# meilisearch/arroy

Hardware: AMD Instinct MI355X
Metric: distances/sec, Q=1 batched 768-dim cosine scan (GB/s vs HBM roofline in `roofline`); tree-build seconds at 10M vectors in `build_10m` (higher is better)
Workload: dtype f32; 1 GPU; 1M x 768 cosine Q=1 scan (configs[1])

## Files before the change

arroy_amd/_lib.py:

```python
from __future__ import annotations

import ctypes as C
import os
import subprocess

HERE = os.path.dirname(os.path.abspath(__file__))
LIB_PATH = os.environ.get("AH_LIB_PATH") or os.path.join(HERE, "libarroy_hip.so")
CSRC = os.path.join(HERE, "csrc")

AH_OK = 0
STATUS_NAMES = {
    1: "InvalidVecDimension", 2: "BuildCancelled", 3: "Panic(device)", 4: "Panic(out of memory)",
    5: "Panic(invalid argument)", 6: "MissingKey", 7: "Panic(not finalized)", 8: "Panic(need preprocess)",
}
AH_SPLIT_SAMPLES = 12


class ArroyHipError(RuntimeError):
    def __init__(self, status: int, message: str, detail=None):
        super().__init__(f"{STATUS_NAMES.get(status, status)}: {message}")
        self.status = status
        self.message = message
        self.item = detail.item if detail is not None else 0
        self.expected = detail.expected if detail is not None else 0
# ... 93 lines not shown

NODE_BATCH_FN = C.CFUNCTYPE(C.c_int, C.c_void_p, C.POINTER(AhNodeBatch))


_VP, _U32P, _F32P, _U64P = C.c_void_p, C.c_void_p, C.c_void_p, C.c_void_p
SIGNATURES = {
    "ah_header_size": (C.c_size_t, [C.c_int]),
    "ah_vector_size": (C.c_size_t, [C.c_int, C.c_uint32]),
    "ah_abi_version": (C.c_int, []),
    "ah_device_count": (C.c_int, [C.POINTER(C.c_int)]),
    "ah_last_error": (C.c_char_p, []),
    "ah_last_error_detail": (C.c_int, [C.POINTER(AhErrorDetail)]),
    "ah_dataset_upload_flush": (C.c_int, [_VP]),
    "ah_dataset_set_preprocessed": (C.c_int, [_VP, C.c_int]),
    "ah_dataset_replicate": (C.c_int, [_VP, C.c_int, C.POINTER(C.c_void_p)]),
    "ah_dataset_create": (C.c_int, [C.c_int, C.c_uint32, C.c_uint64, C.c_int, C.POINTER(C.c_void_p)]),
    "ah_dataset_upload_records": (C.c_int, [_VP, _U32P, _VP, C.c_size_t, C.c_size_t]),
    "ah_dataset_upload_vectors": (C.c_int, [_VP, _U32P, _F32P, C.c_size_t]),
    "ah_dataset_fill_synthetic": (C.c_int, [_VP, C.c_uint64, C.c_int, C.c_uint64]),
    "ah_dataset_finalize": (C.c_int, [_VP]),
    "ah_dataset_reserve_build": (C.c_int, [_VP, C.c_uint32, C.c_uint32]),
    "ah_dataset_rerank_stats": (C.c_int, [_VP, C.POINTER(AhRerankStats), C.c_int]),
    "ah_dataset_packed_info": (C.c_int, [_VP, C.POINTER(C.c_int), C.POINTER(C.c_uint64)]),
    "ah_debug_query_screen_verify": (C.c_int, [_VP, C.POINTER(C.c_uint64), C.POINTER(C.c_uint64), C.c_int]),
    "ah_dataset_len": (C.c_int, [_VP, C.POINTER(C.c_uint64)]),
    "ah_dataset_item_vector": (C.c_int, [_VP, C.c_uint32, _F32P]),
    "ah_dataset_read_headers": (C.c_int, [_VP, C.c_uint64, C.c_uint64, _VP]),
    "ah_dataset_destroy": (C.c_int, [_VP]),
    "ah_preprocess_dot": (C.c_int, [_VP, C.POINTER(C.c_float)]),
    "ah_distances_by_vector": (C.c_int, [_VP, _F32P, _U32P, C.c_size_t, _F32P]),
    "ah_distances_by_item": (C.c_int, [_VP, C.c_uint32, _U32P, C.c_size_t, _F32P]),
    "ah_rerank_by_vector": (C.c_int, [_VP, _F32P, _U32P, C.c_size_t, C.c_size_t, _U32P, _F32P,
                                      C.POINTER(C.c_size_t)]),
    "ah_rerank_by_item": (C.c_int, [_VP, C.c_uint32, _U32P, C.c_size_t, C.c_size_t, _U32P, _F32P,
                                    C.POINTER(C.c_size_t)]),
    "ah_rerank_batch": (C.c_int, [_VP, _F32P, C.c_size_t, _U32P, _U64P, C.c_size_t, _U32P, _F32P, _U32P]),
    "ah_split_sides": (C.c_int, [_VP, _VP, _VP, _U32P, C.c_size_t, _VP, C.POINTER(C.c_uint64), _F32P]),
    "ah_margins": (C.c_int, [_VP, _VP, _VP, _U32P, C.c_size_t, _F32P]),
    "ah_create_split": (C.c_int, [_VP, _U32P, _VP, _VP]),
    "ah_build_forest": (C.c_int, [_VP, C.POINTER(AhBuildOptions), C.POINTER(C.c_void_p)]),
    "ah_build_forest_stream": (C.c_int, [_VP, C.POINTER(AhBuildOptions), NODE_BATCH_FN, _VP, _U32P, C.POINTER(AhBuildStats)]),
    "ah_build_subtrees": (C.c_int, [_VP, C.POINTER(AhBuildOptions), _U32P, _U64P, C.POINTER(C.c_void_p)]),
    "ah_forest_view_get": (C.c_int, [_VP, C.POINTER(AhForestView)]),
    "ah_forest_stats": (C.c_int, [_VP, C.POINTER(AhBuildStats)]),
    "ah_forest_digest": (C.c_int, [_VP, _U64P, C.POINTER(C.c_uint64)]),
    "ah_host_cache_trim": (C.c_int, [C.POINTER(C.c_uint64)]),
# ... 171 lines not shown
```

arroy_amd/csrc/api.hip:

```cpp
#include <algorithm>
#include <atomic>
#include <chrono>
#include <cmath>
#include <condition_variable>
#include <functional>
#include <immintrin.h>
#include <new>
#include <thread>
#include <cctype>
#include <cstdio>
#include <mutex>
#include <vector>
#include <sched.h>
#include <sys/syscall.h>
#include <unistd.h>

#include "common.h"

namespace ah {

static thread_local std::string g_error;
static thread_local ah_error_detail g_detail = {AH_OK, 0, 0, 0};

static thread_local int g_guard_depth = 0;
// ... 2249 lines not shown
    AH_GUARDED_END
}

int ah_dataset_rerank_stats(ah_dataset *ds, ah_rerank_stats *out, int reset) {
    AH_GUARDED("ah_dataset_rerank_stats")
    AH_REQUIRE(ds, AH_ERR_INVALID_ARGUMENT, "dataset is NULL");
    std::lock_guard<std::mutex> lk(ds->mu);
    if (out) *out = ds->rr_stats;
    if (reset) ds->rr_stats = ah_rerank_stats{};
    return AH_OK;
    AH_GUARDED_END
}

int ah_dataset_packed_info(ah_dataset *ds, int *out_present, uint64_t *out_raw_rows) {
    AH_GUARDED("ah_dataset_packed_info")
    AH_REQUIRE(ds, AH_ERR_INVALID_ARGUMENT, "dataset is NULL");
    std::lock_guard<std::mutex> lk(ds->mu);
    if (out_present) *out_present = ds->d_packed ? 1 : 0;
    if (out_raw_rows) *out_raw_rows = ds->d_packed ? ds->packed_raw_rows : 0;
    return AH_OK;
    AH_GUARDED_END
}

int ah_debug_query_screen_verify(ah_dataset *ds, uint64_t *out_checked, uint64_t *out_violations, int reset) {
    AH_GUARDED("ah_debug_query_screen_verify")
    AH_REQUIRE(ds, AH_ERR_INVALID_ARGUMENT, "dataset is NULL");
    DeviceRestore restore;
    std::lock_guard<std::mutex> lk(ds->mu);
    unsigned long long c[2] = {0ull, 0ull};
    if (ds->d_query_verify) {
        AH_HIP(hipSetDevice(ds->device));
        AH_HIP(hipDeviceSynchronize());
        AH_HIP(hipMemcpy(c, ds->d_query_verify, 16, hipMemcpyDeviceToHost));
        if (reset) AH_HIP(hipMemset(ds->d_query_verify, 0, 16));
    }
    if (out_checked) *out_checked = c[0];
    if (out_violations) *out_violations = c[1];
    return AH_OK;
    AH_GUARDED_END
}

int ah_split_sides(ah_dataset *ds, const void *normal_vector, const void *normal_header, const uint32_t *sorted_ids,
                   size_t n, uint8_t *side_bits, uint64_t *out_n_left, float *out_margins) {
    AH_GUARDED("ah_split_sides")
    AH_NEED_FINALIZED(ds);
    AH_REQUIRE(normal_vector && normal_header && side_bits && out_n_left, AH_ERR_INVALID_ARGUMENT, "NULL argument");
// ... 233 lines not shown
```

arroy_amd/csrc/common.h:

```cpp
#pragma once

#include <hip/hip_runtime.h>

#include <cstdarg>
#include <cstdint>
#include <cstdio>
#include <atomic>
#include <cstring>
#include <mutex>
#include <new>
#include <string>
#include <thread>
#include <vector>

#include "../../include/arroy_hip.h"
#include "../../include/arroy_hip_policy.h"

namespace ah {

void set_error(const char *fmt, ...);
const char *last_error();
void set_error_status(int status);
void set_error_detail(uint32_t item, uint64_t expected, uint64_t received);

// ... 74 lines not shown
    X(SCREEN_VERIFY, "AH_SCREEN_VERIFY", 0)       \
    X(NODE_PREFETCH, "AH_NODE_PREFETCH", 1)         \
    X(SCREEN8_LO, "AH_SCREEN8_LO", 1)                 \
    X(SCREEN8, "AH_SCREEN8", -1)                 \
    X(MASK_BITS, "AH_MASK_BITS", -1)             \
    X(DENSE, "AH_DENSE", -1)                        \
    X(DENSE_MAX_COLS, "AH_DENSE_MAX_COLS", 16384)                                                                        \
    X(DENSE_NARROW, "AH_DENSE_NARROW", -1)               \
    X(DENSE_NARROW_MAX_COLS, "AH_DENSE_NARROW_MAX_COLS", 64)    \
    X(DENSE_NARROW_STREAM, "AH_DENSE_NARROW_STREAM", 0)  \
    X(DENSE_GMACS, "AH_DENSE_GMACS", 495000)           \
    X(MARGIN_MODE, "AH_MARGIN_MODE", 0)                          \
    X(READBACK_DIRECT, "AH_READBACK_DIRECT", 0)              \
    X(READBACK_PRIORITY, "AH_READBACK_PRIORITY", 1)  \
    X(READBACK_MB, "AH_READBACK_MB", 256)        \
    X(NUMA, "AH_NUMA", 1)                        \
    X(RETRY_GATE, "AH_RETRY_GATE", 1)            \
    X(TAIL_GROUPS, "AH_BUILD_TAIL_GROUPS", 5)    \
    X(TAIL_MIN_MB, "AH_BUILD_TAIL_MIN_MB", 64)   \
    X(TAIL_NODE_ITEMS, "AH_BUILD_TAIL_NODE_ITEMS", 2)  \
    X(TAIL_RATIO, "AH_BUILD_TAIL_RATIO", 76)     \
    X(SCAN_BLOCKS, "AH_SCAN_BLOCKS", 0)                                 \
    X(SCAN_PACKED, "AH_SCAN_PACKED", -1)         \
    X(MANHATTAN_ROWS, "AH_MANHATTAN_ROWS", 1)                                                                            \
    X(RERANK_INVERT, "AH_RERANK_INVERT", -1)          \
    X(RERANK_SMALL, "AH_RERANK_SMALL", 1)        \
    X(PAIR_GROUP, "AH_PAIR_GROUP", 0)                                                                                    \
    X(PAIR_RUNS, "AH_PAIR_RUNS", 1)                                                                                      \
    X(SEARCH_BITMAP, "AH_SEARCH_BITMAP", 1)          \
    X(SEARCH_TILES, "AH_SEARCH_TILES", 1)                          \
    X(SEARCH_WAVE, "AH_SEARCH_WAVE", 1)                        \
    X(SEARCH_BLOCK_MAX_QUERIES, "AH_SEARCH_BLOCK_MAX_QUERIES", 64)  \
    X(SEARCH_SMALL_GATE, "AH_SEARCH_SMALL_GATE", 1)  \
    X(SEARCH_SMALL_UNITS_MAX_QUERIES, "AH_SEARCH_SMALL_UNITS_MAX_QUERIES", 64)  \
    X(SEARCH_FUSED_FLAG, "AH_SEARCH_FUSED_FLAG", 1)  \
    X(SEARCH_FUSED_PREPARE, "AH_SEARCH_FUSED_PREPARE", 1)  \
    X(SEARCH_SINGLE_FUSED, "AH_SEARCH_SINGLE_FUSED", 1)  \
    X(SEARCH_SMALL_TILES_MAX_QUERIES, "AH_SEARCH_SMALL_TILES_MAX_QUERIES", 8)  \
    X(SEARCH_MULTI, "AH_SEARCH_MULTI", 1)        \
    X(SEARCH_MULTI_TREES_PER_BLOCK, "AH_SEARCH_MULTI_TREES_PER_BLOCK", 8)  \
    X(SEARCH_MULTI_IDS_BY_TILES, "AH_SEARCH_MULTI_IDS_BY_TILES", 1)  \
    X(SEARCH_SPIN_WAIT, "AH_SEARCH_SPIN_WAIT", 1)  \
    X(SEARCH_FLAT_TILES, "AH_SEARCH_FLAT_TILES", 1)  \
    X(SEARCH_STATUS_WIPE, "AH_SEARCH_STATUS_WIPE", 1)  \
    X(SEARCH_ITEM_LIST, "AH_SEARCH_ITEM_LIST", 1)  \
    X(SEARCH_MULTI_OWN_UNITS, "AH_SEARCH_MULTI_OWN_UNITS", 1)  \
// ... 76 lines not shown
    float *headers;
    const uint32_t *ids;
    const uint32_t *lut;
    uint32_t lut_len;
    int identity_ids;
};

struct ScreenView {
    const uint16_t *rows;
    const float4 *stats;
    uint32_t hpitch;
    float gamma_s, gamma_r;
    float4 max_stats;
    const int8_t *rows8;
    uint32_t pitch8;
    const float *scale8_rows;
    float4 max8;
    const int8_t *rows8_lo;
    float4 max8b;
};

static constexpr uint16_t kPackedRaw = 0xFFu;
static constexpr uint16_t kPackedZeros = 0x100u;
struct PackedView {
    const uint8_t *rows = nullptr;
    const uint16_t *row_exp = nullptr;
    uint32_t pitch = 0;
    uint32_t hi_off = 0, code_off = 0;
};
inline PackedView packed_layout(uint32_t dims) {
    const uint32_t b = dims / 32;
    PackedView pk;
    pk.hi_off = 128u * ((b + 1) / 2);
    pk.code_off = pk.hi_off + 128u * ((b + 3) / 4);
    pk.pitch = pk.code_off + 128u * ((b + 7) / 8);
    return pk;
}

struct Context {
    hipStream_t stream = nullptr;
    hipStream_t copy_stream = nullptr;
    hipEvent_t ev0 = nullptr, ev1 = nullptr;
    hipEvent_t ev_t0 = nullptr, ev_t1 = nullptr;
    hipEvent_t ev_ring[4] = {nullptr, nullptr, nullptr, nullptr};
    void *d_scratch = nullptr;
    size_t d_cap = 0;
// ... 51 lines not shown
    double screen8_quality = 0.0;
    uint32_t hpitch = 0;
    bool screen_never = false;
    bool screen8_decided = false;
    bool screen_alloc_failed = false;
    std::atomic<bool> screen_ready{false};
    std::atomic<uint32_t> rerank8_fails{0};
    std::atomic<uint32_t> rerank8_seen{0};
    std::atomic<bool> rerank8_off{false};
    std::atomic<bool> screen8_ready{false};
    ah::Context *up_ctx = nullptr;
    int up_buf = 0;
    bool up_used[4] = {false, false, false, false};
    std::mutex up_mu;
    bool group_member = false;
    std::mutex mu;
    std::vector<ah::Context *> pool;
    bool counted = false;
    std::thread reserve_thread;
    bool replicated_through_host = false;
    uint8_t *d_packed = nullptr;
    uint16_t *d_packed_exp = nullptr;
    uint64_t packed_raw_rows = 0;
    std::atomic<bool> packed_decided{false};
    std::atomic<bool> packed_ready{false};
    unsigned long long *d_query_verify = nullptr;
    ah_rerank_stats rr_stats{};
    double reserve_seconds = 0.0;
    double reserve_wait_seconds = 0.0;
    std::atomic<int> live_indexes{0};
    uint64_t update_fast_paths[3] = {0, 0, 0};

    void join_reserve() {
        std::thread t;
        {
            std::lock_guard<std::mutex> lk(mu);
            t = std::move(reserve_thread);
        }
        if (t.joinable()) {
            try {
                t.join();
            } catch (...) {
            }
        }
    }
    ah::DataView view() const;
// ... 125 lines not shown
```

arroy_amd/csrc/device_math.h:

```cpp
#pragma once

#include <hip/hip_runtime.h>

#include "common.h"

namespace ah {

#pragma clang fp contract(off)
__device__ __forceinline__ float f_add(float a, float b) { return a + b; }
__device__ __forceinline__ float f_sub(float a, float b) { return a - b; }
__device__ __forceinline__ float f_mul(float a, float b) { return a * b; }
__device__ __forceinline__ float f_div(float a, float b) { return a / b; }
__device__ __forceinline__ float f_sqrt(float a) { return sqrtf(a); }

enum { OP_DOT = 0, OP_EUCLID = 1 };

typedef float f32x4_t __attribute__((ext_vector_type(4)));
__device__ __forceinline__ float4 ld_stream(const float4 *p) {
    f32x4_t v = __builtin_nontemporal_load(reinterpret_cast<const f32x4_t *>(p));
    return make_float4(v.x, v.y, v.z, v.w);
}

typedef uint32_t u32x4_t __attribute__((ext_vector_type(4)));
__device__ __forceinline__ uint4 ld_stream_u4(const uint4 *p) {
// ... 188 lines not shown
        const uint32_t o = full;
        const uint4 z = make_uint4(0u, 0u, 0u, 0u);
        uint4 lo[4] = {z, z, z, z}, hi[2] = {z, z};
#pragma unroll
        for (uint32_t u = 0; u < 4; u++)
            if (2 * u < m) lo[u] = ld_stream_u4(lo4 + (4 * o + u) * 8);
#pragma unroll
        for (uint32_t u = 0; u < 2; u++)
            if (4 * u < m) hi[u] = ld_stream_u4(hi4 + (2 * o + u) * 8);
        uint4 nc = ld_stream_u4(c4 + o * 8);
        nc = make_uint4(~nc.x, ~nc.y, ~nc.z, ~nc.w);
        const float4 *bq = b4 + o * 64;
        fma_step<OP>(acc, bq[0], packed_block<ZEROS, 0>(lo, hi, nc, base));
        if (m > 1) fma_step<OP>(acc, bq[8], packed_block<ZEROS, 1>(lo, hi, nc, base));
        if (m > 2) fma_step<OP>(acc, bq[16], packed_block<ZEROS, 2>(lo, hi, nc, base));
        if (m > 3) fma_step<OP>(acc, bq[24], packed_block<ZEROS, 3>(lo, hi, nc, base));
        if (m > 4) fma_step<OP>(acc, bq[32], packed_block<ZEROS, 4>(lo, hi, nc, base));
        if (m > 5) fma_step<OP>(acc, bq[40], packed_block<ZEROS, 5>(lo, hi, nc, base));
        if (m > 6) fma_step<OP>(acc, bq[48], packed_block<ZEROS, 6>(lo, hi, nc, base));
    }
    return octet_finish(acc);
}

template <int OP>
__device__ __forceinline__ float thread_reduce_small(const float *a, const float *b, uint32_t dims) {
    float r = 0.0f;
    uint32_t m = 0;
    if (dims >= 16) {
        m = dims - (dims % 16);
        float c[16];
#pragma unroll
        for (int l = 0; l < 16; l++) c[l] = 0.0f;
        for (uint32_t i = 0; i < m; i += 16) {
#pragma unroll
            for (int l = 0; l < 16; l++) {
                float p;
                if (OP == OP_DOT) {
                    p = f_mul(a[i + l], b[i + l]);
                } else {
                    float s = f_sub(a[i + l], b[i + l]);
                    p = f_mul(s, s);
                }
                c[l] = f_add(p, c[l]);
            }
        }
        float h[4];
// ... 108 lines not shown
```

arroy_amd/csrc/distance.hip:

```cpp
#include <cstdlib>

#include "common.h"
#include "device_math.h"

namespace ah {

static constexpr int kBlock = 256;
static constexpr int kMaxBlocks = 32768;
#define g_max_blocks ((int)(tun(TUN_SCAN_BLOCKS) > 0 ? tun(TUN_SCAN_BLOCKS) : kMaxBlocks))
#define g_manhattan_rows (tun(TUN_MANHATTAN_ROWS) != 0)

static inline unsigned grid_for(uint64_t work_items, int items_per_block) {
    uint64_t b = (work_items + items_per_block - 1) / items_per_block;
    if (b < 1) b = 1;
    if (b > (uint64_t)g_max_blocks) b = g_max_blocks;
    return (unsigned)b;
}

__global__ void k_prepare_query(DataView dv, const float *__restrict__ q_f32, void *qvec, float *qhdr) {
    const uint32_t t = threadIdx.x;
    if (!metric_is_bq_dev(dv.metric)) {
        float *dst = reinterpret_cast<float *>(qvec);
        for (uint32_t i = t; i < dv.pitch; i += blockDim.x) dst[i] = i < dv.dims ? q_f32[i] : 0.0f;
        __syncthreads();
// ... 65 lines not shown

    const uint32_t j = threadIdx.x & 7u;
    const uint64_t n_octets = ((uint64_t)gridDim.x * blockDim.x) >> 3;
    for (uint64_t i = ((uint64_t)blockIdx.x * blockDim.x + threadIdx.x) >> 3; i < n; i += n_octets) {
        uint64_t row = i;
        if (GATHER) {
            row = row_of_id(dv, ids[i]);
            if (row == ~0ull) {
                if (j == 0) {
                    atomicOr(err, 1u);
                    out[i] = __uint_as_float(0x7FC00000u);
                }
                continue;
            }
            if (i > 0 && ids[i] <= ids[i - 1] && j == 0) atomicOr(err, 2u);
        }
        const float *rp = dv.rows_f32 + row * dv.pitch;
        float r;
        if (METRIC == AH_MANHATTAN) {
            r = octet_manhattan(s_q, rp, dv.dims, j);
        } else if constexpr (PACKED) {
            const uint32_t ex = pk.row_exp[row];
            const uint8_t *pr = pk.rows + row * pk.pitch;
            if (ex == kPackedRaw)
                r = octet_reduce_stream<OP>(s_q4, rp, dv.dims, j);
            else if (ex & kPackedZeros)
                r = octet_reduce_packed<OP, true>(s_q4, pr, pk.hi_off, pk.code_off, dv.dims >> 5, ex & 0xFFu, j);
            else
                r = octet_reduce_packed<OP, false>(s_q4, pr, pk.hi_off, pk.code_off, dv.dims >> 5, ex, j);
        } else {
            r = octet_reduce_stream<OP>(s_q4, rp, dv.dims, j);
        }
        if (j == 0) out[i] = f32_epilogue<METRIC>(r, s_hdr, dv, row);
    }
}

template <int METRIC, bool GATHER>
__global__ __launch_bounds__(kBlock) void k_distances_f32(DataView dv, PackedView pk, const float *__restrict__ qvec,
                                                          const float *__restrict__ qhdr,
                                                          const uint32_t *__restrict__ ids, uint64_t n,
                                                          float *__restrict__ out, uint32_t *err) {
    extern __shared__ float4 s_q4[];
    __shared__ float s_hdr[2];
    f32_scan<METRIC, GATHER, !GATHER>(dv, pk, s_q4, s_hdr, qvec, qhdr, ids, n, out, err);
}
template <int METRIC>
__global__ __launch_bounds__(kBlock) void k_distances_f32_rows(DataView dv, const float *__restrict__ qvec,
// ... 281 lines not shown
        const unsigned g = grid_for(n, kBlock);
#define AH_LAUNCH_SMALL(M)                                                                                      \
    hipLaunchKernelGGL((k_distances_f32_small<M, GATHER>), dim3(g), dim3(kBlock), 0, s, dv, (const float *)qvec, \
                       qhdr, ids, n, out, err)
        switch (dv.metric) {
        case AH_EUCLIDEAN: AH_LAUNCH_SMALL(AH_EUCLIDEAN); break;
        case AH_MANHATTAN: AH_LAUNCH_SMALL(AH_MANHATTAN); break;
        case AH_COSINE: AH_LAUNCH_SMALL(AH_COSINE); break;
        default: AH_LAUNCH_SMALL(AH_DOT_PRODUCT); break;
        }
#undef AH_LAUNCH_SMALL
    }
    AH_HIP(hipGetLastError());
    return AH_OK;
}

int launch_distances(const DataView &dv, const void *d_qvec, const float *d_qhdr, const uint32_t *d_ids, uint64_t n,
                     float *d_out, uint32_t *d_err, hipStream_t s, const PackedView &pk) {
    return d_ids ? launch_distances_t<true>(dv, d_qvec, d_qhdr, d_ids, n, d_out, d_err, s, PackedView{})
                 : launch_distances_t<false>(dv, d_qvec, d_qhdr, nullptr, n, d_out, d_err, s, pk);
}

__global__ __launch_bounds__(kBlock) void k_pack_rows(DataView dv, uint8_t *__restrict__ rows, uint16_t *__restrict__ row_exp,
                                                      PackedView lay, unsigned long long *raw_rows) {
    const uint32_t j = threadIdx.x & 7u;
    const uint32_t blocks = dv.dims >> 5;
    const uint64_t n_octets = ((uint64_t)gridDim.x * blockDim.x) >> 3;
    uint32_t raw_here = 0;
    for (uint64_t r = ((uint64_t)blockIdx.x * blockDim.x + threadIdx.x) >> 3; r < dv.n; r += n_octets) {
        const float4 *src = reinterpret_cast<const float4 *>(dv.rows_f32 + r * dv.pitch) + j;
        uint32_t emax = 0, emin = 255, special = 0, zeros = 0;
        for (uint32_t k = 0; k < blocks; k++) {
            const float4 x = src[k * 8];
            const float v[4] = {x.x, x.y, x.z, x.w};
#pragma unroll
            for (int i = 0; i < 4; i++) {
                const uint32_t e = (__float_as_uint(v[i]) >> 23) & 255u;
                emax = max(emax, e);
                if (e != 0u) emin = min(emin, e);
                special |= e == 255u;
                zeros |= e == 0u;
            }
        }
#pragma unroll
        for (int m = 1; m < 8; m <<= 1) {
            emax = max(emax, (uint32_t)__shfl_xor((int)emax, m));
            emin = min(emin, (uint32_t)__shfl_xor((int)emin, m));
            special |= (uint32_t)__shfl_xor((int)special, m);
            zeros |= (uint32_t)__shfl_xor((int)zeros, m);
        }
        const bool raw = special || (int)emax - (int)emin >= 15;
        if (j == 0) row_exp[r] = raw ? kPackedRaw : (uint16_t)(emax | (zeros ? kPackedZeros : 0u));
        if (raw) {
            raw_here += j == 0;
            continue;
        }
        uint8_t *dst = rows + r * lay.pitch;
        for (uint32_t o = 0; o < (blocks + 7) / 8; o++) {
            uint32_t lo[16], hi[8], cd[4];
#pragma unroll
            for (int w = 0; w < 16; w++) lo[w] = 0u;
#pragma unroll
            for (int w = 0; w < 8; w++) hi[w] = 0u;
#pragma unroll
            for (int w = 0; w < 4; w++) cd[w] = 0u;
#pragma unroll
            for (int t = 0; t < 8; t++) {
                const uint32_t k = 8 * o + t;
                const float4 x = k < blocks ? src[k * 8] : make_float4(0.f, 0.f, 0.f, 0.f);
                const float v[4] = {x.x, x.y, x.z, x.w};
#pragma unroll
                for (int i = 0; i < 4; i++) {
                    const uint32_t b = __float_as_uint(v[i]);
                    const uint32_t e = (b >> 23) & 255u;
                    const uint32_t c = e == 0u ? 15u : emax - e;
                    const int u = (t & 1) * 4 + i;
                    lo[(t >> 1) * 4 + u / 2] |= (b & 0xFFFFu) << (16 * (u & 1));
                    hi[t] |= (((b >> 24) & 0x80u) | ((b >> 16) & 0x7Fu)) << (8 * i);
                    cd[t >> 1] |= c << (4 * u);
                }
            }
            uint4 *lo4 = reinterpret_cast<uint4 *>(dst) + j;
            uint4 *hi4 = reinterpret_cast<uint4 *>(dst + lay.hi_off) + j;
            uint4 *c4 = reinterpret_cast<uint4 *>(dst + lay.code_off) + j;
#pragma unroll
            for (uint32_t u = 0; u < 4; u++)
                if (8 * o + 2 * u < blocks) lo4[(4 * o + u) * 8] = make_uint4(lo[4 * u], lo[4 * u + 1], lo[4 * u + 2], lo[4 * u + 3]);
#pragma unroll
            for (uint32_t u = 0; u < 2; u++)
                if (8 * o + 4 * u < blocks) hi4[(2 * o + u) * 8] = make_uint4(hi[4 * u], hi[4 * u + 1], hi[4 * u + 2], hi[4 * u + 3]);
            c4[o * 8] = make_uint4(cd[0], cd[1], cd[2], cd[3]);
        }
    }
    if (raw_here) atomicAdd(raw_rows, (unsigned long long)raw_here);
}

static int launch_pack_rows(const DataView &dv, uint8_t *rows, uint16_t *row_exp, const PackedView &lay,
                            unsigned long long *d_raw, hipStream_t s) {
    const unsigned grid = (unsigned)std::min<uint64_t>((dv.n + 31) / 32, 1u << 16);
    hipLaunchKernelGGL(k_pack_rows, dim3(grid), dim3(kBlock), 0, s, dv, rows, row_exp, lay, d_raw);
    AH_HIP(hipGetLastError());
    return AH_OK;
}

static constexpr uint64_t kPackedMinRows = 65536;
static bool packed_pays(uint32_t dims) { return 16ull * (packed_layout(dims).pitch + 2) <= 15ull * 4 * dims; }
PackedView ensure_packed(ah_dataset *ds, hipStream_t s) {
    const long long mode = tun(TUN_SCAN_PACKED);
    if (mode == 0) return PackedView{};
    PackedView pk = packed_layout(ds->dims);
    if (!ds->packed_ready.load(std::memory_order_acquire)) {
        if (ds->metric != AH_COSINE && ds->metric != AH_EUCLIDEAN && ds->metric != AH_DOT_PRODUCT) return PackedView{};
        if (ds->dims < 32 || ds->dims % 32 != 0 || ds->n == 0) return PackedView{};
        if (mode != 1 && (ds->packed_decided.load(std::memory_order_acquire) || ds->n < kPackedMinRows || !packed_pays(ds->dims)))
            return PackedView{};
        std::lock_guard<std::mutex> lk(ds->mu);
        if (!ds->d_packed) {
            if (mode != 1 && ds->packed_decided.load(std::memory_order_relaxed)) return PackedView{};
            ds->packed_decided.store(true, std::memory_order_release);
            uint8_t *rows = nullptr;
            uint16_t *row_exp = nullptr;
            unsigned long long *d_raw = nullptr, h_raw = 0;
            bool ok = dev_malloc((void **)&rows, ds->n * (size_t)pk.pitch, true) == hipSuccess &&
                      dev_malloc((void **)&row_exp, ds->n * 2, true) == hipSuccess &&
                      dev_malloc((void **)&d_raw, 8, true) == hipSuccess && hipMemsetAsync(d_raw, 0, 8, s) == hipSuccess;
            ok = ok && launch_pack_rows(ds->view(), rows, row_exp, pk, d_raw, s) == AH_OK;
            ok = ok && hipMemcpyAsync(&h_raw, d_raw, 8, hipMemcpyDeviceToHost, s) == hipSuccess;
            ok = hipStreamSynchronize(s) == hipSuccess && ok;
            ok = ok && (mode == 1 || h_raw <= ds->n / 4);
            if (d_raw) (void)dev_free(d_raw);
            if (!ok) {
                (void)hipGetLastError();
                if (rows) (void)dev_free(rows);
                if (row_exp) (void)dev_free(row_exp);
                return PackedView{};
            }
            ds->d_packed = rows;
            ds->d_packed_exp = row_exp;
            ds->packed_raw_rows = h_raw;
            ds->packed_ready.store(true, std::memory_order_release);
        }
    }
    pk.rows = ds->d_packed;
    pk.row_exp = ds->d_packed_exp;
    return pk;
}

int launch_prepare_query(const DataView &dv, const float *d_query_f32, void *d_qvec, float *d_qhdr, hipStream_t s) {
    hipLaunchKernelGGL(k_prepare_query, dim3(1), dim3(metric_is_bq_dev(dv.metric) ? 64 : 1024), 0, s, dv, d_query_f32, d_qvec, d_qhdr);
    AH_HIP(hipGetLastError());
    return AH_OK;
}
int launch_load_item_as_query(const DataView &dv, uint32_t row, void *d_qvec, float *d_qhdr, hipStream_t s) {
    hipLaunchKernelGGL(k_load_item_as_query, dim3(1), dim3(64), 0, s, dv, row, d_qvec, d_qhdr);
    AH_HIP(hipGetLastError());
    return AH_OK;
}

static constexpr uint32_t kChunk = 4096;
static constexpr uint64_t kSentinel = ~0ull;

__device__ __forceinline__ uint64_t make_key(float d, uint64_t pos, uint32_t id, uint64_t two_k) {
// ... 468 lines not shown
```

arroy_amd/csrc/update.hip:

```cpp
#include <algorithm>
#include <chrono>
#include <vector>

#include "common.h"

using namespace ah;

namespace {

constexpr unsigned kUpBlock = 256;
constexpr uint32_t kScanPer = 16;
constexpr uint32_t kScanTile = kUpBlock * kScanPer;
enum Path { kInPlace = 0, kAppend = 1, kMerge = 2 };
const char *const kPathName[3] = {"in place", "append", "merge"};

unsigned grid_of(uint64_t work, uint64_t per_block, unsigned cap) {
    return (unsigned)std::max<uint64_t>(1, std::min<uint64_t>((work + per_block - 1) / per_block, cap));
}

__device__ __forceinline__ uint64_t lower_bound_u32(const uint32_t *a, uint64_t n, uint32_t x) {
    uint64_t lo = 0, hi = n;
    while (lo < hi) {
        const uint64_t mid = (lo + hi) >> 1;
        if (a[mid] < x) lo = mid + 1;
// ... 414 lines not shown
        ds->last_id = p.last_id;
        ds->identity_ids = p.identity;
    }
    ds->screen_ready.store(false, std::memory_order_release);
    ds->screen8_ready.store(false, std::memory_order_release);
    ds->packed_ready.store(false, std::memory_order_release);
    free_copy(ds->d_rows_h16);
    free_copy(ds->d_screen_stats);
    free_copy(ds->d_rows_i8);
    free_copy(ds->d_rows_i8_lo);
    free_copy(ds->d_scale8_rows);
    free_copy(ds->d_dim_scale);
    free_copy(ds->d_packed);
    free_copy(ds->d_packed_exp);
    std::fill(std::begin(ds->screen_max), std::end(ds->screen_max), 0.0f);
    std::fill(std::begin(ds->screen8_max), std::end(ds->screen8_max), 0.0f);
    ds->hpitch = 0;
    ds->pitch8 = 0;
    ds->screen8_quality = 0.0;
    ds->screen_never = false;
    ds->screen8_decided = false;
    ds->screen_alloc_failed = false;
    ds->packed_raw_rows = 0;
    ds->packed_decided.store(false, std::memory_order_release);
    ds->rerank8_fails.store(0, std::memory_order_relaxed);
    ds->rerank8_seen.store(0, std::memory_order_relaxed);
    ds->rerank8_off.store(false, std::memory_order_relaxed);
    ds->rr_stats = ah_rerank_stats{};
    if (ds->metric == AH_DOT_PRODUCT) ds->dot_preprocessed = false;
    ds->update_fast_paths[p.path]++;
}

int update_impl(const std::vector<ah_dataset *> &members, ah_group *g, const UpdateArgs &a) {
    auto now = [] { return std::chrono::steady_clock::now(); };
    const auto t0 = now();
    ah_dataset *ds0 = members[0];
    for (ah_dataset *m : members) {
        AH_TRY(flush_staging(m));
        AH_TRY(check_member(m));
    }
    AH_TRY(check_sorted(a.rm, a.n_rm, "remove_ids"));
    AH_TRY(check_sorted(a.up, a.n_up, "upsert_ids"));
    AH_REQUIRE(a.n_up == 0 || a.vectors || a.records, AH_ERR_INVALID_ARGUMENT, "the upserted items are NULL");
    const Plan p = make_plan(ds0, a);
    AH_REQUIRE(p.n_new < 0xFFFFFFFFull, AH_ERR_INVALID_ARGUMENT, "the update exceeds the u32 item-id space");
    DeviceRestore restore_device;
// ... 112 lines not shown
```

arroy_amd/dataset.py:

```python
from __future__ import annotations

import ctypes as C
from typing import Optional, Sequence

import numpy as np

from . import _lib
from .distances import BY_METRIC, Distance


def _u32(a) -> np.ndarray:
    return np.ascontiguousarray(a, dtype=np.uint32)


def _f32(a) -> np.ndarray:
    return np.ascontiguousarray(a, dtype=np.float32)


def _ptr(a: Optional[np.ndarray]):
    return None if a is None else a.ctypes.data_as(C.c_void_p)


def _update_rows(dimensions: int, up: np.ndarray, vectors) -> Optional[np.ndarray]:
    if up.size == 0:
# ... 141 lines not shown
        if isinstance(id_lists, tuple):
            ids, offsets = _u32(id_lists[0]), np.ascontiguousarray(id_lists[1], dtype=np.uint64)
            assert offsets.size == nq + 1 and int(offsets[-1]) == ids.size
        else:
            offsets = np.zeros(nq + 1, dtype=np.uint64)
            offsets[1:] = np.cumsum([len(l) for l in id_lists])
            ids = _u32(np.concatenate([_u32(l) for l in id_lists])) if nq else np.zeros(0, np.uint32)
        oi = np.zeros((nq, k), dtype=np.uint32)
        od = np.zeros((nq, k), dtype=np.float32)
        oc = np.zeros(nq, dtype=np.uint32)
        _lib.check(_lib.lib().ah_rerank_batch(self._h, _ptr(q), nq, _ptr(ids), _ptr(offsets), k, _ptr(oi), _ptr(od),
                                              _ptr(oc)))
        return oi, od, oc

    def rerank_stats(self, reset: bool = False) -> dict:
        st = _lib.AhRerankStats()
        _lib.check(_lib.lib().ah_dataset_rerank_stats(self._h, C.byref(st), 1 if reset else 0))
        return {f: getattr(st, f) for f, _ in _lib.AhRerankStats._fields_}

    def packed_info(self) -> dict:
        present, raw = C.c_int(0), C.c_uint64(0)
        _lib.check(_lib.lib().ah_dataset_packed_info(self._h, C.byref(present), C.byref(raw)))
        return {"present": bool(present.value), "raw_rows": raw.value}

    def query_screen_verify(self, reset: bool = False) -> dict:
        checked, bad = C.c_uint64(0), C.c_uint64(0)
        _lib.check(_lib.lib().ah_debug_query_screen_verify(self._h, C.byref(checked), C.byref(bad), 1 if reset else 0))
        return {"checked": checked.value, "violations": bad.value}

    def split_sides(self, normal_vector: np.ndarray, normal_header, sorted_ids=None, want_margins: bool = True):
        ids_a = None if sorted_ids is None else _u32(sorted_ids)
        n = len(self) if ids_a is None else ids_a.size
        nv = np.ascontiguousarray(normal_vector).view(np.uint8)
        assert nv.size == self.distance.vector_size(self.dimensions)
        nh = np.zeros(2, dtype=np.float32)
        h = _f32(normal_header).ravel()
        nh[: h.size] = h
        bits = np.zeros((n + 7) // 8, dtype=np.uint8)
        margins = np.zeros(n, dtype=np.float32) if want_margins else None
        nl = C.c_uint64(0)
        _lib.check(_lib.lib().ah_split_sides(self._h, _ptr(nv), _ptr(nh), _ptr(ids_a), n, _ptr(bits), C.byref(nl),
                                             _ptr(margins)))
        sides = np.unpackbits(bits, bitorder="little")[:n]
        return sides, int(nl.value), margins

    def create_split(self, sample_ids: Sequence[int]):
# ... 481 lines not shown
```

include/arroy_hip.h:

```cpp
#ifndef ARROY_HIP_H
#define ARROY_HIP_H

#include <stddef.h>
#include <stdint.h>

#ifdef __cplusplus
extern "C" {
#endif

#define AH_ABI_VERSION 7

#if defined(__GNUC__)
#define AH_API __attribute__((visibility("default")))
#else
#define AH_API
#endif

typedef enum ah_metric {
    AH_EUCLIDEAN = 0,
    AH_MANHATTAN = 1,
    AH_COSINE = 2,
    AH_DOT_PRODUCT = 3,
    AH_BQ_EUCLIDEAN = 4,
    AH_BQ_MANHATTAN = 5,
// ... 65 lines not shown
                        uint32_t *out_ids, float *out_distances, size_t *out_n);
AH_API int ah_rerank_by_item(ah_dataset *ds, uint32_t query_item, const uint32_t *sorted_ids, size_t n, size_t k,
                      uint32_t *out_ids, float *out_distances, size_t *out_n);
AH_API int ah_rerank_batch(ah_dataset *ds, const float *queries, size_t n_queries, const uint32_t *ids,
                    const uint64_t *offsets, size_t k, uint32_t *out_ids, float *out_distances,
                    uint32_t *out_counts);

typedef struct ah_rerank_stats {
    uint64_t calls;
    uint64_t queries, candidates;
    double seconds_wall;
    double seconds_prep;
    double seconds_ids;
    double seconds_enqueue;
    double seconds_sync_wait;
    double seconds_device_span;
    uint64_t queries_screened;
    uint64_t survivors;
    uint64_t chunks_int8;
    uint64_t chunks_int8_retried;
} ah_rerank_stats;
AH_API int ah_dataset_rerank_stats(ah_dataset *ds, ah_rerank_stats *out, int reset);
AH_API int ah_dataset_packed_info(ah_dataset *ds, int *out_present, uint64_t *out_raw_rows);
AH_API int ah_debug_query_screen_verify(ah_dataset *ds, uint64_t *out_checked, uint64_t *out_violations, int reset);


#define AH_SPLIT_SAMPLES 12

AH_API int ah_split_sides(ah_dataset *ds, const void *normal_vector, const void *normal_header,
                   const uint32_t *sorted_ids, size_t n, uint8_t *side_bits, uint64_t *out_n_left,
                   float *out_margins);

AH_API int ah_margins(ah_dataset *normals, const void *leaf_vector, const void *leaf_header, const uint32_t *item_ids,
                      size_t n, float *out_margins);

AH_API int ah_create_split(ah_dataset *ds, const uint32_t sample_ids[AH_SPLIT_SAMPLES], void *out_normal_vector,
                    void *out_normal_header);

typedef void (*ah_progress_fn)(void *user, uint32_t level, uint64_t nodes_done, uint64_t items_routed);

typedef enum ah_margin_mode {
    AH_MARGIN_AUTO = 0,
    AH_MARGIN_NODE_MAJOR = 1,
    AH_MARGIN_ROWS_2 = 2,
    AH_MARGIN_ROWS_4 = 4,
    AH_MARGIN_ROWS_8 = 8,
// ... 216 lines not shown
```

Before: 2.582 billion distances/s.

## Add lossless fixed-point grid packing for rows whose mantissas fit 24 bits

Adds a new packed row format. It is used for rows whose every value lies exactly on a fixed-point grid set by the row's maximum exponent: no specials, no denormals, and low set bit at or above emax+1. Each value is stored as a 16-bit low word plus an 8-bit sign/high byte, 3 bytes in place of 4, and decoded on the scan path with perm/bfi plus one subtract against a 2^(emax+1) bias. The aim is to cut the HBM bytes read per row in the streaming cosine scan without losing accuracy, at the cost of extra ALU decode work and a more expensive pack kernel. Whether it pays off depends on how many dataset rows meet the grid condition; typical float embeddings may rarely do so.

```diff
diff --git a/arroy_amd/_lib.py b/arroy_amd/_lib.py
--- a/arroy_amd/_lib.py
+++ b/arroy_amd/_lib.py
@@ -139,6 +139,7 @@
     "ah_dataset_reserve_build": (C.c_int, [_VP, C.c_uint32, C.c_uint32]),
     "ah_dataset_rerank_stats": (C.c_int, [_VP, C.POINTER(AhRerankStats), C.c_int]),
     "ah_dataset_packed_info": (C.c_int, [_VP, C.POINTER(C.c_int), C.POINTER(C.c_uint64)]),
+    "ah_dataset_packed_rows": (C.c_int, [_VP, C.POINTER(C.c_int), C.POINTER(C.c_uint64), C.POINTER(C.c_uint64)]),
     "ah_debug_query_screen_verify": (C.c_int, [_VP, C.POINTER(C.c_uint64), C.POINTER(C.c_uint64), C.c_int]),
     "ah_dataset_len": (C.c_int, [_VP, C.POINTER(C.c_uint64)]),
     "ah_dataset_item_vector": (C.c_int, [_VP, C.c_uint32, _F32P]),
diff --git a/arroy_amd/csrc/api.hip b/arroy_amd/csrc/api.hip
--- a/arroy_amd/csrc/api.hip
+++ b/arroy_amd/csrc/api.hip
@@ -2295,6 +2295,17 @@
     AH_GUARDED_END
 }
 
+int ah_dataset_packed_rows(ah_dataset *ds, int *out_present, uint64_t *out_raw_rows, uint64_t *out_grid_rows) {
+    AH_GUARDED("ah_dataset_packed_rows")
+    AH_REQUIRE(ds, AH_ERR_INVALID_ARGUMENT, "dataset is NULL");
+    std::lock_guard<std::mutex> lk(ds->mu);
+    if (out_present) *out_present = ds->d_packed ? 1 : 0;
+    if (out_raw_rows) *out_raw_rows = ds->d_packed ? ds->packed_raw_rows : 0;
+    if (out_grid_rows) *out_grid_rows = ds->d_packed ? ds->packed_grid_rows : 0;
+    return AH_OK;
+    AH_GUARDED_END
+}
+
 int ah_debug_query_screen_verify(ah_dataset *ds, uint64_t *out_checked, uint64_t *out_violations, int reset) {
     AH_GUARDED("ah_debug_query_screen_verify")
     AH_REQUIRE(ds, AH_ERR_INVALID_ARGUMENT, "dataset is NULL");
diff --git a/arroy_amd/csrc/common.h b/arroy_amd/csrc/common.h
--- a/arroy_amd/csrc/common.h
+++ b/arroy_amd/csrc/common.h
@@ -120,6 +120,7 @@
     X(TAIL_RATIO, "AH_BUILD_TAIL_RATIO", 76)     \
     X(SCAN_BLOCKS, "AH_SCAN_BLOCKS", 0)                                 \
     X(SCAN_PACKED, "AH_SCAN_PACKED", -1)         \
+    X(SCAN_GRID, "AH_SCAN_GRID", 1)              \
     X(MANHATTAN_ROWS, "AH_MANHATTAN_ROWS", 1)                                                                            \
     X(RERANK_INVERT, "AH_RERANK_INVERT", -1)          \
     X(RERANK_SMALL, "AH_RERANK_SMALL", 1)        \
@@ -242,6 +243,8 @@
 
 static constexpr uint16_t kPackedRaw = 0xFFu;
 static constexpr uint16_t kPackedZeros = 0x100u;
+static constexpr uint16_t kPackedGrid = 0x200u;
+static constexpr uint32_t kGridMinExp = 25u, kGridMaxExp = 253u;
 struct PackedView {
     const uint8_t *rows = nullptr;
     const uint16_t *row_exp = nullptr;
@@ -339,6 +342,7 @@
     uint8_t *d_packed = nullptr;
     uint16_t *d_packed_exp = nullptr;
     uint64_t packed_raw_rows = 0;
+    uint64_t packed_grid_rows = 0;
     std::atomic<bool> packed_decided{false};
     std::atomic<bool> packed_ready{false};
     unsigned long long *d_query_verify = nullptr;
diff --git a/arroy_amd/csrc/device_math.h b/arroy_amd/csrc/device_math.h
--- a/arroy_amd/csrc/device_math.h
+++ b/arroy_amd/csrc/device_math.h
@@ -234,6 +234,74 @@
     return octet_finish(acc);
 }
 
+template <uint32_t SEL>
+__device__ __forceinline__ float grid_value(uint32_t lo, uint32_t hi, uint32_t two) {
+    const uint32_t a = __builtin_amdgcn_perm(hi, lo, SEL);
+    uint32_t r, s;
+    asm("v_bfi_b32 %0, %1, %2, %3" : "=v"(r) : "s"(0x007FFFFFu), "v"(a), "v"(two));
+    const float f = f_sub(__uint_as_float(r), __uint_as_float(two));
+    asm("v_bfi_b32 %0, %1, %2, %3" : "=v"(s) : "s"(0x80000000u), "v"(a), "v"(__float_as_uint(f)));
+    return __uint_as_float(s);
+}
+template <int T>
+__device__ __forceinline__ float4 grid_block(const uint4 (&lo)[4], const uint4 (&hi)[2], uint32_t two) {
+    constexpr int P = T & 1;
+    const uint4 l = lo[T >> 1];
+    const uint32_t l0 = P ? l.z : l.x, l1 = P ? l.w : l.y;
+    const uint4 h = hi[T >> 2];
+    const uint32_t hw = (T & 3) == 0 ? h.x : (T & 3) == 1 ? h.y : (T & 3) == 2 ? h.z : h.w;
+    return make_float4(grid_value<0x04040100u>(l0, hw, two), grid_value<0x05050302u>(l0, hw, two),
+                       grid_value<0x06060100u>(l1, hw, two), grid_value<0x07070302u>(l1, hw, two));
+}
+template <int OP>
+__device__ __forceinline__ float octet_reduce_packed_grid(const float4 *s_b4, const uint8_t *prow, uint32_t hi_off, uint32_t blocks,
+                                                          uint32_t emax, uint32_t j) {
+    const uint4 *lo4 = reinterpret_cast<const uint4 *>(prow) + j;
+    const uint4 *hi4 = reinterpret_cast<const uint4 *>(prow + hi_off) + j;
+    const float4 *b4 = s_b4 + j;
+    const uint32_t two = (emax + 1u) << 23;
+    float4 acc = make_float4(0.f, 0.f, 0.f, 0.f);
+    const uint32_t full = blocks / 8;
+#pragma unroll 1
+    for (uint32_t o = 0; o < full; o++) {
+        uint4 lo[4], hi[2];
+#pragma unroll
+        for (int u = 0; u < 4; u++) lo[u] = ld_stream_u4(lo4 + (4 * o + u) * 8);
+#pragma unroll
+        for (int u = 0; u < 2; u++) hi[u] = ld_stream_u4(hi4 + (2 * o + u) * 8);
+        const float4 *bq = b4 + o * 64;
+        fma_step<OP>(acc, bq[0], grid_block<0>(lo, hi, two));
+        fma_step<OP>(acc, bq[8], grid_block<1>(lo, hi, two));
+        fma_step<OP>(acc, bq[16], grid_block<2>(lo, hi, two));
+        fma_step<OP>(acc, bq[24], grid_block<3>(lo, hi, two));
+        fma_step<OP>(acc, bq[32], grid_block<4>(lo, hi, two));
+        fma_step<OP>(acc, bq[40], grid_block<5>(lo, hi, two));
+        fma_step<OP>(acc, bq[48], grid_block<6>(lo, hi, two));
+        fma_step<OP>(acc, bq[56], grid_block<7>(lo, hi, two));
+    }
+    const uint32_t m = blocks - 8 * full;
+    if (m) {
+        const uint32_t o = full;
+        const uint4 z = make_uint4(0u, 0u, 0u, 0u);
+        uint4 lo[4] = {z, z, z, z}, hi[2] = {z, z};
+#pragma unroll
+        for (uint32_t u = 0; u < 4; u++)
+            if (2 * u < m) lo[u] = ld_stream_u4(lo4 + (4 * o + u) * 8);
+#pragma unroll
+        for (uint32_t u = 0; u < 2; u++)
+            if (4 * u < m) hi[u] = ld_stream_u4(hi4 + (2 * o + u) * 8);
+        const float4 *bq = b4 + o * 64;
+        fma_step<OP>(acc, bq[0], grid_block<0>(lo, hi, two));
+        if (m > 1) fma_step<OP>(acc, bq[8], grid_block<1>(lo, hi, two));
+        if (m > 2) fma_step<OP>(acc, bq[16], grid_block<2>(lo, hi, two));
+        if (m > 3) fma_step<OP>(acc, bq[24], grid_block<3>(lo, hi, two));
+        if (m > 4) fma_step<OP>(acc, bq[32], grid_block<4>(lo, hi, two));
+        if (m > 5) fma_step<OP>(acc, bq[40], grid_block<5>(lo, hi, two));
+        if (m > 6) fma_step<OP>(acc, bq[48], grid_block<6>(lo, hi, two));
+    }
+    return octet_finish(acc);
+}
+
 template <int OP>
 __device__ __forceinline__ float thread_reduce_small(const float *a, const float *b, uint32_t dims) {
     float r = 0.0f;
diff --git a/arroy_amd/csrc/distance.hip b/arroy_amd/csrc/distance.hip
--- a/arroy_amd/csrc/distance.hip
+++ b/arroy_amd/csrc/distance.hip
@@ -111,7 +111,9 @@
         } else if constexpr (PACKED) {
             const uint32_t ex = pk.row_exp[row];
             const uint8_t *pr = pk.rows + row * pk.pitch;
-            if (ex == kPackedRaw)
+            if (ex & kPackedGrid)
+                r = octet_reduce_packed_grid<OP>(s_q4, pr, pk.hi_off, dv.dims >> 5, ex & 0xFFu, j);
+            else if (ex == kPackedRaw)
                 r = octet_reduce_stream<OP>(s_q4, rp, dv.dims, j);
             else if (ex & kPackedZeros)
                 r = octet_reduce_packed<OP, true>(s_q4, pr, pk.hi_off, pk.code_off, dv.dims >> 5, ex & 0xFFu, j);
@@ -439,24 +441,27 @@
 }
 
 __global__ __launch_bounds__(kBlock) void k_pack_rows(DataView dv, uint8_t *__restrict__ rows, uint16_t *__restrict__ row_exp,
-                                                      PackedView lay, unsigned long long *raw_rows) {
+                                                      PackedView lay, int grid, unsigned long long *counts) {
     const uint32_t j = threadIdx.x & 7u;
     const uint32_t blocks = dv.dims >> 5;
     const uint64_t n_octets = ((uint64_t)gridDim.x * blockDim.x) >> 3;
-    uint32_t raw_here = 0;
+    uint32_t raw_here = 0, grid_here = 0;
     for (uint64_t r = ((uint64_t)blockIdx.x * blockDim.x + threadIdx.x) >> 3; r < dv.n; r += n_octets) {
         const float4 *src = reinterpret_cast<const float4 *>(dv.rows_f32 + r * dv.pitch) + j;
-        uint32_t emax = 0, emin = 255, special = 0, zeros = 0;
+        uint32_t emax = 0, emin = 255, special = 0, zeros = 0, lowbit = 0xFFFFu, denormal = 0;
         for (uint32_t k = 0; k < blocks; k++) {
             const float4 x = src[k * 8];
             const float v[4] = {x.x, x.y, x.z, x.w};
 #pragma unroll
             for (int i = 0; i < 4; i++) {
-                const uint32_t e = (__float_as_uint(v[i]) >> 23) & 255u;
+                const uint32_t b = __float_as_uint(v[i]);
+                const uint32_t e = (b >> 23) & 255u;
                 emax = max(emax, e);
                 if (e != 0u) emin = min(emin, e);
                 special |= e == 255u;
                 zeros |= e == 0u;
+                if (e != 0u) lowbit = min(lowbit, e + (uint32_t)__builtin_ctz(b | 0x800000u));
+                denormal |= e == 0u && (b & 0x7FFFFFu) != 0u;
             }
         }
 #pragma unroll
@@ -465,6 +470,44 @@
             emin = min(emin, (uint32_t)__shfl_xor((int)emin, m));
             special |= (uint32_t)__shfl_xor((int)special, m);
             zeros |= (uint32_t)__shfl_xor((int)zeros, m);
+            lowbit = min(lowbit, (uint32_t)__shfl_xor((int)lowbit, m));
+            denormal |= (uint32_t)__shfl_xor((int)denormal, m);
+        }
+        uint8_t *dst = rows + r * lay.pitch;
+        if (grid && !special && !denormal && emax >= kGridMinExp && emax <= kGridMaxExp && lowbit >= emax + 1u) {
+            if (j == 0) row_exp[r] = (uint16_t)(emax | kPackedGrid);
+            grid_here += j == 0;
+            for (uint32_t o = 0; o < (blocks + 7) / 8; o++) {
+                uint32_t lo[16], hi[8];
+#pragma unroll
+                for (int w = 0; w < 16; w++) lo[w] = 0u;
+#pragma unroll
+                for (int w = 0; w < 8; w++) hi[w] = 0u;
+#pragma unroll
+                for (int t = 0; t < 8; t++) {
+                    const uint32_t k = 8 * o + t;
+                    const float4 x = k < blocks ? src[k * 8] : make_float4(0.f, 0.f, 0.f, 0.f);
+                    const float v[4] = {x.x, x.y, x.z, x.w};
+#pragma unroll
+                    for (int i = 0; i < 4; i++) {
+                        const uint32_t b = __float_as_uint(v[i]);
+                        const uint32_t e = (b >> 23) & 255u;
+                        const uint32_t mag = e == 0u ? 0u : ((b & 0x7FFFFFu) | 0x800000u) >> ((emax - e + 1u) & 31u);
+                        const int u = (t & 1) * 4 + i;
+                        lo[(t >> 1) * 4 + u / 2] |= (mag & 0xFFFFu) << (16 * (u & 1));
+                        hi[t] |= (((b >> 24) & 0x80u) | (mag >> 16)) << (8 * i);
+                    }
+                }
+                uint4 *lo4 = reinterpret_cast<uint4 *>(dst) + j;
+                uint4 *hi4 = reinterpret_cast<uint4 *>(dst + lay.hi_off) + j;
+#pragma unroll
+                for (uint32_t u = 0; u < 4; u++)
+                    if (8 * o + 2 * u < blocks) lo4[(4 * o + u) * 8] = make_uint4(lo[4 * u], lo[4 * u + 1], lo[4 * u + 2], lo[4 * u + 3]);
+#pragma unroll
+                for (uint32_t u = 0; u < 2; u++)
+                    if (8 * o + 4 * u < blocks) hi4[(2 * o + u) * 8] = make_uint4(hi[4 * u], hi[4 * u + 1], hi[4 * u + 2], hi[4 * u + 3]);
+            }
+            continue;
         }
         const bool raw = special || (int)emax - (int)emin >= 15;
         if (j == 0) row_exp[r] = raw ? kPackedRaw : (uint16_t)(emax | (zeros ? kPackedZeros : 0u));
@@ -472,7 +515,6 @@
             raw_here += j == 0;
             continue;
         }
-        uint8_t *dst = rows + r * lay.pitch;
         for (uint32_t o = 0; o < (blocks + 7) / 8; o++) {
             uint32_t lo[16], hi[8], cd[4];
 #pragma unroll
@@ -509,13 +551,14 @@
             c4[o * 8] = make_uint4(cd[0], cd[1], cd[2], cd[3]);
         }
     }
-    if (raw_here) atomicAdd(raw_rows, (unsigned long long)raw_here);
-}
-
-static int launch_pack_rows(const DataView &dv, uint8_t *rows, uint16_t *row_exp, const PackedView &lay,
-                            unsigned long long *d_raw, hipStream_t s) {
+    if (raw_here) atomicAdd(counts, (unsigned long long)raw_here);
+    if (grid_here) atomicAdd(counts + 1, (unsigned long long)grid_here);
+}
+
+static int launch_pack_rows(const DataView &dv, uint8_t *rows, uint16_t *row_exp, const PackedView &lay, bool grid_rows,
+                            unsigned long long *d_counts, hipStream_t s) {
     const unsigned grid = (unsigned)std::min<uint64_t>((dv.n + 31) / 32, 1u << 16);
-    hipLaunchKernelGGL(k_pack_rows, dim3(grid), dim3(kBlock), 0, s, dv, rows, row_exp, lay, d_raw);
+    hipLaunchKernelGGL(k_pack_rows, dim3(grid), dim3(kBlock), 0, s, dv, rows, row_exp, lay, grid_rows ? 1 : 0, d_counts);
     AH_HIP(hipGetLastError());
     return AH_OK;
 }
@@ -537,13 +580,15 @@
             ds->packed_decided.store(true, std::memory_order_release);
             uint8_t *rows = nullptr;
             uint16_t *row_exp = nullptr;
-            unsigned long long *d_raw = nullptr, h_raw = 0;
+            unsigned long long *d_raw = nullptr, h_counts[2] = {0, 0};
+            const bool grid_rows = tun(TUN_SCAN_GRID) != 0;
             bool ok = dev_malloc((void **)&rows, ds->n * (size_t)pk.pitch, true) == hipSuccess &&
                       dev_malloc((void **)&row_exp, ds->n * 2, true) == hipSuccess &&
-                      dev_malloc((void **)&d_raw, 8, true) == hipSuccess && hipMemsetAsync(d_raw, 0, 8, s) == hipSuccess;
-            ok = ok && launch_pack_rows(ds->view(), rows, row_exp, pk, d_raw, s) == AH_OK;
-            ok = ok && hipMemcpyAsync(&h_raw, d_raw, 8, hipMemcpyDeviceToHost, s) == hipSuccess;
+                      dev_malloc((void **)&d_raw, 16, true) == hipSuccess && hipMemsetAsync(d_raw, 0, 16, s) == hipSuccess;
+            ok = ok && launch_pack_rows(ds->view(), rows, row_exp, pk, grid_rows, d_raw, s) == AH_OK;
+            ok = ok && hipMemcpyAsync(h_counts, d_raw, 16, hipMemcpyDeviceToHost, s) == hipSuccess;
             ok = hipStreamSynchronize(s) == hipSuccess && ok;
+            const unsigned long long h_raw = h_counts[0];
             ok = ok && (mode == 1 || h_raw <= ds->n / 4);
             if (d_raw) (void)dev_free(d_raw);
             if (!ok) {
@@ -555,6 +600,7 @@
             ds->d_packed = rows;
             ds->d_packed_exp = row_exp;
             ds->packed_raw_rows = h_raw;
+            ds->packed_grid_rows = h_counts[1];
             ds->packed_ready.store(true, std::memory_order_release);
         }
     }
diff --git a/arroy_amd/csrc/update.hip b/arroy_amd/csrc/update.hip
--- a/arroy_amd/csrc/update.hip
+++ b/arroy_amd/csrc/update.hip
@@ -460,6 +460,7 @@
     ds->screen8_decided = false;
     ds->screen_alloc_failed = false;
     ds->packed_raw_rows = 0;
+    ds->packed_grid_rows = 0;
     ds->packed_decided.store(false, std::memory_order_release);
     ds->rerank8_fails.store(0, std::memory_order_relaxed);
     ds->rerank8_seen.store(0, std::memory_order_relaxed);
diff --git a/arroy_amd/dataset.py b/arroy_amd/dataset.py
--- a/arroy_amd/dataset.py
+++ b/arroy_amd/dataset.py
@@ -187,6 +187,11 @@
         present, raw = C.c_int(0), C.c_uint64(0)
         _lib.check(_lib.lib().ah_dataset_packed_info(self._h, C.byref(present), C.byref(raw)))
         return {"present": bool(present.value), "raw_rows": raw.value}
+
+    def packed_rows(self) -> dict:
+        present, raw, grid = C.c_int(0), C.c_uint64(0), C.c_uint64(0)
+        _lib.check(_lib.lib().ah_dataset_packed_rows(self._h, C.byref(present), C.byref(raw), C.byref(grid)))
+        return {"present": bool(present.value), "raw_rows": raw.value, "grid_rows": grid.value}
 
     def query_screen_verify(self, reset: bool = False) -> dict:
         checked, bad = C.c_uint64(0), C.c_uint64(0)
diff --git a/include/arroy_hip.h b/include/arroy_hip.h
--- a/include/arroy_hip.h
+++ b/include/arroy_hip.h
@@ -111,6 +111,7 @@
 } ah_rerank_stats;
 AH_API int ah_dataset_rerank_stats(ah_dataset *ds, ah_rerank_stats *out, int reset);
 AH_API int ah_dataset_packed_info(ah_dataset *ds, int *out_present, uint64_t *out_raw_rows);
+AH_API int ah_dataset_packed_rows(ah_dataset *ds, int *out_present, uint64_t *out_raw_rows, uint64_t *out_grid_rows);
 AH_API int ah_debug_query_screen_verify(ah_dataset *ds, uint64_t *out_checked, uint64_t *out_violations, int reset);
 
 
```

New measurement: 3.071 billion distances/s (median of 6 runs). 1.19x the previous value.
